# CVlab315/Domain-Adaptative-Hand-Pose-Estimation

Hardware: AMD Instinct MI355X
Metric: images/sec (unique source+target images per A+B+C training iteration, 2*B*N/t_iter) (higher is better)
Workload: dtype bf16; 1 GPU; RHD->H3D domain-adaptation iteration (steps A+B+C), resnet50 + 3-deconv neck + main head + 3 adversarial multiscale-fusion heads, 256x256, batch 64 source + 64 target per GPU, random init, synthetic batches; arch=resnet50, image_size=256, per_gpu_batch=64, global_batch=64, parallelism=dp1, hip_graphs=True, gradient_exchange=none (one rank)

## Files before the change

domain-adaptative-hand-pose-estimation_amd/csrc/conv_plan.h:

```cpp
#pragma once
#include <stdlib.h>
#include "common.h"

#define MAX_TAPS 52
struct Tap { int8_t dy, dx; int16_t widx; };

struct Phase { int OHp, OWp, out_oy, out_ox, M, ntaps, tap0, ntm; };
struct GatherArgs {
  const void* A; const void* B; void* D;
  const float* bias; const void* residual; const float* scale;
  int Hi, Wi, Ci;
  int in_sy, in_sx;
  int Ho, Wo;
  int out_sy, out_sx;
  int Nout, ldb, ldd;
  int cshift;
  int accumulate;
  int nphase, ntn, ntiles;
  int hw;
  int lw;
  unsigned a_bytes, b_bytes;
  size_t stat_bytes;
  int stat_slices;
  const void* bnb_x; const void* bnb_y;
// ... 12 lines not shown
  const float* bias2;
  int c2;
  union { unsigned a2_bytes; unsigned mx_sa_bytes; };
  union { unsigned b2_bytes; unsigned mx_sb_bytes; };
  int pg_nadd;
  int mx_act;
  void* mx_y8; void* mx_sy;
};

inline long conv_knob(const char* name, long dflt, bool* set = nullptr) {
  const char* v = getenv(name);
  if (set) *set = v != nullptr;
  return v ? atol(v) : dflt;
}
inline bool conv_knob_set(const char* name) { bool set; (void)conv_knob(name, 0, &set); return set; }
struct ConvKnobs {
  int tile = (int)conv_knob("MI355_TILE", -1);
  int dma = (int)conv_knob("MI355_DMA", 1);
  int cat_tile = (int)conv_knob("MI355_CAT_TILE", 0);
  int t256d = (int)conv_knob("MI355_T256D", 2);
  long t256d_min = conv_knob("MI355_T256D_MIN", 192);
  long t256d_kmin = conv_knob("MI355_T256D_KMIN", 32);
  bool t256 = conv_knob_set("MI355_T256");
  int kw3 = (int)conv_knob("MI355_KW3", 1);
  int kw3_n64 = (int)conv_knob("MI355_KW3_N64", 1);
  int splitk = (int)conv_knob("MI355_SPLITK", 2);
  long splitk_min = conv_knob("MI355_SPLITK_MIN", 128), splitk_max = conv_knob("MI355_SPLITK_MAX", 320);
  long splitk_kmin = conv_knob("MI355_SPLITK_KMIN", 128);
  bool stats256 = conv_knob("MI355_STATS_256", 1) != 0;
  int phases = (int)conv_knob("MI355_PHASES", 1);
  int wg_blocks = (int)conv_knob("MI355_WG_BLOCKS", 768);
  int wgrad_kw = (int)conv_knob("MI355_WGRAD_KW", 1);
  int wgrad_kw2 = (int)conv_knob("MI355_WGRAD_KW2", 1);
  bool wgrad_group256 = conv_knob("MI355_WGRAD_GROUP256", 1) != 0;
  bool wgrad_kw_group = conv_knob("MI355_WGRAD_KW_GROUP", 1) != 0;
  int wg_group_blocks = (int)conv_knob("MI355_WG_GROUP_BLOCKS", 512);
  int wg_group256_blocks = (int)conv_knob("MI355_WG_GROUP256_BLOCKS", 256);
  int wg_kw_group_blocks = (int)conv_knob("MI355_WG_KW_GROUP_BLOCKS", 512);
  int pgemm = (int)conv_knob("MI355_PGEMM", 1), pgemm_set = -1;
  int pg_add_maxk = (int)conv_knob("MI355_PG_ADD", 1) * 64;
  long pg_min_rows = conv_knob("MI355_PG_MIN_ROWS", 32768);
  int pg_ring = (int)conv_knob("MI355_PG_RING", 0), pg_bm = (int)conv_knob("MI355_PG_BM", 64);
  int pg_per_cu = (int)conv_knob("MI355_PG_PER_CU", 2);
  int fp8_tile = (int)conv_knob("MI355_FP8_TILE", -1);
  long fp8_kw3 = conv_knob("MI355_FP8_KW3", 1024), fp8_kw3_set = -1;
};
inline ConvKnobs& conv_knobs() { static ConvKnobs k; return k; }

static inline void describe_fwd(GatherArgs& a, const mi355_conv_desc* d) {
  a.Hi = d->Hi; a.Wi = d->Wi; a.Ci = d->Ci; a.in_sy = a.in_sx = d->stride;
  a.Ho = d->Ho; a.Wo = d->Wo; a.out_sy = a.out_sx = 1;
  a.Nout = d->Co; a.ldd = d->Co; a.ldb = d->kh * d->kw * d->Ci;
  a.nphase = 1; a.ph[0].OHp = d->Ho; a.ph[0].OWp = d->Wo; a.ph[0].M = d->N * d->Ho * d->Wo; a.ph[0].ntaps = d->kh * d->kw;
  for (int i = 0; i < d->kh; ++i)
    for (int j = 0; j < d->kw; ++j) { Tap& t = a.taps[i * d->kw + j]; t.dy = (int8_t)(i - d->pad); t.dx = (int8_t)(j - d->pad); t.widx = (int16_t)(i * d->kw + j); }
}
static inline bool describe_dgrad(GatherArgs& a, const mi355_conv_desc* d) {
  const int s = d->stride;
  auto parity_without_tap = [&](int k) {
    for (int p = 0; p < s; ++p) { int cnt = 0; for (int i = 0; i < k; ++i) if ((p + d->pad - i) % s == 0) ++cnt; if (!cnt) return true; }
    return false;
  };
  const bool need_zero = parity_without_tap(d->kh) || parity_without_tap(d->kw);
  a.Hi = d->Ho; a.Wi = d->Wo; a.Ci = d->Co;
  a.in_sy = a.in_sx = 1; a.Ho = d->Hi; a.Wo = d->Wi; a.out_sy = a.out_sx = s;
  a.Nout = d->Ci; a.ldd = d->Ci; a.ldb = d->kh * d->kw * d->Co;
// ... 226 lines not shown
constexpr bool gather_has_bnb(int bm, bool hm, bool kw3, bool cat, int kg) { return !hm && bm <= 128 && !kw3 && !cat && kg == 1; }
constexpr bool gather_has_stats(int bm, int bn, bool hm, bool dma) { return !hm && (bm <= 128 || (bm == 256 && bn == 128) || (bm == 256 && bn == 256 && dma)); }
static inline int gather_epilogue(GatherArgs& a, const ConvBuild& b, const ConvKnobs& k) {
  if (!gather_has_bnb(b.bm, b.hm, b.kw3, b.cat, b.kg)) a.bnb_partial = nullptr;
  if (!gather_has_stats(b.bm, b.bn, b.hm, b.dma) || (b.bm == 256 && !k.stats256)) a.stat_partial = nullptr;
  if (!a.stat_partial && !a.bnb_partial) a.stat_slices = 0;
  return a.bnb_partial ? 2 : a.stat_partial ? 1 : 0;
}

static inline void plan_gather_launch(GatherArgs& a, ConvBuild& b, const ConvKnobs& k) {
  plan_tile_grid(a, b.bm, b.bn, b.hm);
  b.epi = b.family == CONV_GATHER ? gather_epilogue(a, b, k) : (b.family == CONV_MX && a.mx_act) ? 3 : (a.stat_partial ? 1 : 0);
  if (b.kw3) a.lw = ilog2_exact(a.Wi);
}

struct WgradSplit { int S, rows; };
static inline WgradSplit wgrad_split(long M, int kstep, long want) {
  const long ksteps = (M + kstep - 1) / kstep;
  long S = want > ksteps ? ksteps : want;
  if (S < 1) S = 1;
  long rps = (M + S - 1) / S; rps = ((rps + kstep - 1) / kstep) * kstep;
  WgradSplit r; r.S = (int)((M + rps - 1) / rps); r.rows = (int)rps;
  return r;
}
static inline WgradSplit wgrad_split_alone(long M, int kstep, long tiles, const ConvKnobs& k) {
  const long ksteps = (M + kstep - 1) / kstep;
  long S = (k.wg_blocks + tiles - 1) / tiles;
  const long S16 = ksteps / 16, S256 = (256 + tiles - 1) / tiles, lo = S16 > S256 ? S16 : S256;
  if (S > lo) S = lo;
  if (tiles >= 384) S = 1;
  return wgrad_split(M, kstep, S);
}

struct WgradPlan { int S, rows_per_split, nto, nti, ldw, kw3, mt, kw2; };
static inline WgradPlan plan_wgrad(const mi355_conv_desc* d, const ConvKnobs& k) {
  WgradPlan w; w.ldw = d->kh * d->kw * d->Ci;
  const int bkm = d->dtype == MI355_BF16 ? 64 : 32;
  const long M = (long)d->N * d->Ho * d->Wo;
  w.kw3 = k.wgrad_kw && d->dtype == MI355_BF16 && d->kh == 3 && d->kw == 3 && d->stride == 1 && d->pad == 1 &&
          d->Ho == d->Hi && d->Wo == d->Wi &&
          d->Wi >= 8 && ilog2_exact(d->Wi) >= 0;
  w.mt = d->Co <= 64 ? 1 : 2;
  w.kw2 = k.wgrad_kw2 && d->dtype == MI355_BF16 && d->kh == d->kw && (d->kh == 3 || d->kh == 4) && d->stride == 2 && d->pad == 1 &&
          d->Hi % 2 == 0 && d->Wi % 2 == 0 && d->Ho == d->Hi / 2 && d->Wo == d->Wi / 2 && d->Wo >= 8 && d->Wo <= 64 &&
          ilog2_exact(d->Wo) >= 0;
  long tiles;
  if (w.kw2) { w.nto = cdiv(d->Co, 64 * w.mt); w.nti = cdiv(d->Ci, 64); tiles = (long)w.nto * d->kh * w.nti; }
  else if (w.kw3) { w.nto = cdiv(d->Co, 64 * w.mt); w.nti = cdiv(d->Ci, 64); tiles = (long)w.nto * 3 * w.nti; }
  else { w.nto = cdiv(d->Co, 128); w.nti = cdiv(w.ldw, 128); tiles = (long)w.nto * w.nti; }
  const WgradSplit s = wgrad_split_alone(M, bkm, tiles, k);
  w.S = s.S; w.rows_per_split = s.rows;
  return w;
}
static inline const char* wgrad_kernel_name(const WgradPlan& w) { return w.kw2 ? "wgrad_kw2" : w.kw3 ? "wgrad_kw" : "wgrad"; }

#define WG_MAX 24
#define WGK_MAX 16
static inline bool group_eligible(const mi355_conv_desc* d, const WgradPlan& w) {
  return !w.kw2 && !w.kw3 && (long)w.nto * w.nti < 384;
}
static inline bool group256_eligible(const mi355_conv_desc* d, const WgradPlan& w) {
  return conv_knobs().wgrad_group256 && d->dtype == MI355_BF16 && d->kh == 1 && d->kw == 1 && d->pad == 0 && d->Co % 256 == 0 && d->Ci % 256 == 0;
}
static inline bool kw_group_eligible(const mi355_conv_desc* d, const WgradPlan& w) {
  if (!conv_knobs().wgrad_kw_group || !w.kw3) return false;
  const long M = (long)d->N * d->Ho * d->Wo, ksteps = (M + 63) / 64;
  return (long)w.nto * 3 * w.nti * ksteps < 768L * 24;
}
static inline long group_tiles(int kind, const mi355_conv_desc* d, const WgradPlan& w) {
  return kind == 3 ? (long)(d->Co / 256) * (w.ldw / 256) : kind == 2 ? (long)w.nto * 3 * w.nti : (long)w.nto * w.nti;
}
struct GroupPlan { int S, rps; size_t ws_off; };
static inline long group_plan(const mi355_wgrad_item* items, const int* idx, int n, GroupPlan* gp, size_t* ws_bytes, int kind) {
  const ConvKnobs& kn = conv_knobs();
  const int target = kind == 3 ? kn.wg_group256_blocks : kind == 2 ? kn.wg_kw_group_blocks : kn.wg_group_blocks;
  auto rows = [](const mi355_conv_desc* d) { return (long)d->N * d->Ho * d->Wo; };
  auto kstep = [](const mi355_conv_desc* d) { return d->dtype == MI355_BF16 ? 64 : 32; };
  double W = 0;
  for (int k = 0; k < n; ++k) {
    const mi355_conv_desc* d = &items[idx[k]].d;
    W += (double)group_tiles(kind, d, plan_wgrad(d, kn)) * ((rows(d) + kstep(d) - 1) / kstep(d));
  }
  long per = (long)(W / target) + 1; if (per < 16) per = 16;
  auto plan_at = [&](long per, GroupPlan* out, size_t* ws_end) {
    long blocks = 0; size_t off = 0;
    for (int k = 0; k < n; ++k) {
      const mi355_wgrad_item& it = items[idx[k]]; const mi355_conv_desc* d = &it.d; const WgradPlan w = plan_wgrad(d, kn);
      const WgradSplit s = wgrad_split(rows(d), kstep(d), ((rows(d) + kstep(d) - 1) / kstep(d) + per - 1) / per);
      if (out) { out[k].S = s.S; out[k].rps = s.rows; out[k].ws_off = off; }
      if (s.S > 1 || it.accumulate) off += (size_t)s.S * d->Co * w.ldw * sizeof(float);
      blocks += group_tiles(kind, d, w) * s.S;
    }
    if (ws_end) *ws_end = off;
    return blocks;
  };
  for (int trial = 0; kind == 3 && trial < 64; ++trial) {
    if (plan_at(per, nullptr, nullptr) <= target) break;
    per += per / 16 + 1;
  }
  return plan_at(per, gp, ws_bytes);
}
template <typename F>
static inline int walk_wgrad_groups(const mi355_wgrad_item* items, int n, F&& fn) {
  int gi[WG_MAX], ki[WGK_MAX], bi[WG_MAX]; int gm = 0, km = 0, bm = 0;
  auto flush_g = [&]() -> int { if (!gm) return 0; int e = fn(1, gi, gm); gm = 0; return e; };
  auto flush_k = [&]() -> int { if (!km) return 0; int e = fn(2, ki, km); km = 0; return e; };
  auto flush_b = [&]() -> int { if (!bm) return 0; int e = fn(3, bi, bm); bm = 0; return e; };
  for (int i = 0; i < n; ++i) {
    const mi355_wgrad_item& it = items[i];
    WgradPlan w = plan_wgrad(&it.d, conv_knobs());
    bool shares = false;
    for (int k = 0; k < gm; ++k) shares = shares || items[gi[k]].dw == it.dw;
    for (int k = 0; k < km; ++k) shares = shares || items[ki[k]].dw == it.dw;
    for (int k = 0; k < bm; ++k) shares = shares || items[bi[k]].dw == it.dw;
    if (shares) { if (int e = flush_g()) return e; if (int e = flush_k()) return e; if (int e = flush_b()) return e; }
    if (kw_group_eligible(&it.d, w)) {
      if (km && (km == WGK_MAX || plan_wgrad(&items[ki[0]].d, conv_knobs()).mt != w.mt)) { if (int e = flush_k()) return e; }
      ki[km++] = i;
    } else if (group_eligible(&it.d, w) && group256_eligible(&it.d, w)) {
      if (bm == WG_MAX) { if (int e = flush_b()) return e; }
      bi[bm++] = i;
    } else if (group_eligible(&it.d, w)) {
      if (gm && (gm == WG_MAX || items[gi[0]].d.dtype != it.d.dtype)) { if (int e = flush_g()) return e; }
      gi[gm++] = i;
    } else {
      int one = i;
      if (int e = fn(0, &one, 1)) return e;
    }
  }
  if (int e = flush_g()) return e;
  if (int e = flush_b()) return e;
  return flush_k();
}
```

domain-adaptative-hand-pose-estimation_amd/csrc/igemm.hip:

```cpp
#include "common.h"
#include <stdlib.h>

#include "igemm_common.h"

template <typename T> struct MmaTraits;
template <> struct MmaTraits<bf16_t> { static constexpr int BK = 64; static constexpr int CH = 8; };
template <> struct MmaTraits<float> { static constexpr int BK = 32; static constexpr int CH = 4; };

#define GATHER_STAGES 1
template <typename T, int BM, int BN, int STAGES = 1, bool KW3 = false>
struct GatherSmem {
  static constexpr int kARows = KW3 ? BM + 4 * (BM / 8) + 4 : BM;
  static constexpr int kStage = (kARows + BN) * 128;
  static constexpr int kOutStride = BN * (int)sizeof(T) + 16;
  static constexpr int kOut = BM * kOutStride;
  static constexpr int kBytes = (STAGES * kStage > kOut ? STAGES * kStage : kOut) + BM * 4;
};

template <typename T, int BM, int BN, bool SMALL_C, int WGM = 2, int WGN = 2, bool HM_OUT = false, bool DMA = false, int EPI = 0,
          bool KW3 = false, bool CAT = false, int KG = 1>
__global__ __launch_bounds__(64 * WGM * WGN * KG, (KW3 && BM == 256) ? 2 : 1) void gather_gemm_kernel(const GatherArgs p) {
  constexpr int CH = MmaTraits<T>::CH;
  constexpr int GTHR = 64 * WGM * WGN;
  constexpr int NTHR = GTHR * KG, RPP = GTHR / 8;
// ... 829 lines not shown
    const unsigned st = smem_lds + (unsigned)((it & 1) * STAGE);
    __builtin_amdgcn_s_setprio(1);
    wg256_step<0>(st, trA, trB, acc); wg256_step<4096>(st, trA, trB, acc); wg256_step<8192>(st, trA, trB, acc); wg256_step<12288>(st, trA, trB, acc);
    __builtin_amdgcn_s_setprio(0);
  }
  float* out = p.out + (size_t)split * p.slab_stride;
#pragma unroll
  for (int i = 0; i < 4; ++i)
#pragma unroll
    for (int j = 0; j < 2; ++j)
#pragma unroll
      for (int r = 0; r < 16; ++r) {
        const int o = o0 + wo * 128 + i * 32 + (r & 3) + 8 * (r >> 2) + 4 * hi;
        const int c = c0 + (wc >> 1) * 128 + wn0 + j * 32 + r31;
        if (o < p.Co && c < p.ldw) out[(size_t)o * p.ldw + c] = acc[i][j][r];
      }
}
__global__ __launch_bounds__(512, 1) void wgrad_group256_kernel(const WgradGroupArgs g) {
  extern __shared__ __attribute__((aligned(16))) char smem256[];
  int i = 0;
  while (i + 1 < g.n && (int)blockIdx.x >= g.bstart[i + 1]) ++i;
  wgrad_gemm256_body(g.p[i], (int)blockIdx.x - g.bstart[i], g.bstart[i + 1] - g.bstart[i], smem256);
}

struct SlabItem { const float* slabs; float* out; long n4, stride; int S, accumulate; };
struct SlabGroupArgs { SlabItem it[WG_MAX]; int bstart[WG_MAX + 1]; int n; };
__global__ __launch_bounds__(256) void slab_reduce_group_kernel(const SlabGroupArgs g) {
  int i = 0;
  while (i + 1 < g.n && (int)blockIdx.x >= g.bstart[i + 1]) ++i;
  const SlabItem& q = g.it[i];
  const long c = (long)((int)blockIdx.x - g.bstart[i]) * 256 + threadIdx.x;
  if (c >= q.n4) return;
  float4 v = make_float4(0.f, 0.f, 0.f, 0.f);
  for (int s = 0; s < q.S; ++s) {
    const float4 a = reinterpret_cast<const float4*>(q.slabs + (size_t)s * q.stride)[c];
    v.x += a.x; v.y += a.y; v.z += a.z; v.w += a.w;
  }
  if (q.accumulate) { const float4 o = reinterpret_cast<const float4*>(q.out)[c]; v.x += o.x; v.y += o.y; v.z += o.z; v.w += o.w; }
  reinterpret_cast<float4*>(q.out)[c] = v;
}

struct WgradKwArgs {
  const void* X; const void* DY; float* out;
  int H, W, Ci, Co;
  int lw, lwf, halo;
  int M, rows_per_split, ldw;
  long slab_stride;
  int nto, nci;
  unsigned x_bytes, dy_bytes;
  FastDiv dH;
};
__device__ __forceinline__ int swzx(int r, int ch) { return r * 128 + ((ch ^ (((r >> 1) & 1) << 2)) << 4); }

template <int MT> struct WgradKwSmem { static constexpr int kBytes = 64 * 256 + (64 + 4 * 8 + 4) * 128 + 2 * 64 * 4; };
template <int MT>
__device__ __forceinline__ void wgrad_kw_body(const WgradKwArgs& p, const int bid, const int nblk, char* smem) {
  constexpr int BO = 64 * MT, BKM = 64;
  constexpr int CPRY = BO / 8, RPY = 256 / CPRY, NPY = BKM / RPY;
  constexpr int XROWS = 64 + 4 * 8 + 4;
  char* ys = smem;
  char* xs = smem + BKM * 256;
  int* rowinfo = reinterpret_cast<int*>(smem + BKM * 256 + XROWS * 128);

  const int t = threadIdx.x, lane = t & 63, wave = t >> 6;
  const int ntile = p.nto * 3 * p.nci;
  const int lid = xcd_remap(bid, nblk);
  const int split = lid / ntile;
// ... 103 lines not shown
        b[k] = __builtin_shufflevector(b0, b1, 0, 1, 2, 3, 4, 5, 6, 7);
      }
#pragma unroll
      for (int k = 0; k < 3; ++k)
#pragma unroll
        for (int i = 0; i < MT; ++i) acc[k][i] = __builtin_amdgcn_mfma_f32_32x32x16_bf16(a[i], b[k], acc[k][i], 0, 0, 0);
    }
    __builtin_amdgcn_s_setprio(0);
  }
  float* out = p.out + (size_t)split * p.slab_stride;
#pragma unroll
  for (int k = 0; k < 3; ++k)
#pragma unroll
    for (int i = 0; i < MT; ++i)
#pragma unroll
      for (int r = 0; r < 16; ++r) {
        const int o = o0 + wm0 + i * 32 + (r & 3) + 8 * (r >> 2) + 4 * hi;
        const int c = ci0 + wn0 + r31;
        if (o < p.Co && c < p.Ci) out[(size_t)o * p.ldw + (kh * 3 + k) * p.Ci + c] = acc[k][i][r];
      }
}
template <int MT>
__global__ __launch_bounds__(256, 3) void wgrad_kw_kernel(const WgradKwArgs p) {
  __shared__ __attribute__((aligned(16))) char smem[WgradKwSmem<MT>::kBytes];
  wgrad_kw_body<MT>(p, (int)blockIdx.x, (int)gridDim.x, smem);
}
struct WgradKwGroupArgs { WgradKwArgs p[WGK_MAX]; int bstart[WGK_MAX + 1]; int n; };
template <int MT>
__global__ __launch_bounds__(256, 3) void wgrad_kw_group_kernel(const WgradKwGroupArgs g) {
  __shared__ __attribute__((aligned(16))) char smem[WgradKwSmem<MT>::kBytes];
  int i = 0;
  while (i + 1 < g.n && (int)blockIdx.x >= g.bstart[i + 1]) ++i;
  wgrad_kw_body<MT>(g.p[i], (int)blockIdx.x - g.bstart[i], g.bstart[i + 1] - g.bstart[i], smem);
}

struct WgradKw2Args {
  const void* X; const void* DY; float* out;
  int H, W, Ho, Ci, Co;
  int lw, lwo;
  int M, rows_per_split, ldw;
  long slab_stride;
  int nto, nci;
  unsigned x_bytes, dy_bytes;
  FastDiv dHo;
};

template <int MT, int KW>
__global__ __launch_bounds__(256, KW == 4 ? 2 : 3) void wgrad_kw2_kernel(const WgradKw2Args p) {
  constexpr int BO = 64 * MT, BKM = 64;
  constexpr int CPRY = BO / 8, RPY = 256 / CPRY, NPY = BKM / RPY;
  constexpr int XROWS = 64 + 4 * 8 + 4;
  __shared__ __attribute__((aligned(16))) char smem[BKM * 256 + 2 * XROWS * 128 + 2 * BKM * 8];
  char* ys = smem;
  char* xe = smem + BKM * 256;
  char* xo = xe + XROWS * 128;
  int2* rowinfo = reinterpret_cast<int2*>(smem + BKM * 256 + 2 * XROWS * 128);

  const int t = threadIdx.x, lane = t & 63, wave = t >> 6;
  const int ntile = p.nto * KW * p.nci;
  const int lid = xcd_remap(blockIdx.x, gridDim.x);
  const int split = lid / ntile;
  int tile = lid - split * ntile;
  const int ot = tile / (KW * p.nci); tile -= ot * KW * p.nci;
  const int kh = tile / p.nci, cit = tile - kh * p.nci;
  const int o0 = ot * BO, ci0 = cit * 64, tdy = kh - 1;
  const int wm0 = (wave >> 1) * (32 * MT), wn0 = (wave & 1) * 32;
// ... 558 lines not shown
}
static int check_wgrad_channels(const mi355_conv_desc* d) {
  const int CH = d->dtype == MI355_BF16 ? 8 : 4;
  if (d->Ci % CH || d->Co % CH) MI_FAIL(MI355_EINVAL, "wgrad: channels must be multiples of %d", CH);
  if (ilog2_exact(d->Ci / CH) < 0) MI_FAIL(MI355_EINVAL, "wgrad: Ci/%d must be a power of two", CH);
  return MI355_OK;
}

extern "C" size_t mi355_conv_wgrad_workspace(const mi355_conv_desc* d) {
  WgradPlan w = plan_wgrad(d, conv_knobs());
  return (size_t)w.S * d->Co * w.ldw * sizeof(float);
}

extern "C" int mi355_conv_wgrad(const mi355_conv_desc* d, const void* x, const void* dy, float* dw, int accumulate,
                                void* ws, size_t ws_bytes, void* stream) {
  if (int e = check_desc(d, true)) return e;
  hipStream_t st = as_stream(stream);
  if (int e = check_wgrad_channels(d)) return e;
  const WgradPlan w = plan_wgrad(d, conv_knobs());
  const size_t need = (size_t)w.S * d->Co * w.ldw * sizeof(float);
  const bool direct = (w.S == 1 && !accumulate);
  if (!direct && (ws == nullptr || ws_bytes < need)) MI_FAIL(MI355_EWORKSPACE, "wgrad workspace %zu < %zu", ws_bytes, need);
  float* out = direct ? dw : reinterpret_cast<float*>(ws);
  const long M = (long)d->N * d->Ho * d->Wo, slab = (long)d->Co * w.ldw, esz = d->dtype == MI355_BF16 ? 2 : 4;
  const unsigned x_bytes = (unsigned)((long)d->N * d->Hi * d->Wi * d->Ci * esz), dy_bytes = (unsigned)(M * d->Co * esz);
  {
    if (prof_on()) prof_set_tag("%s k%ds%d %d>%d @%dx%d n%d S%d", wgrad_kernel_name(w), d->kh, d->stride, d->Ci, d->Co, d->Hi, d->Wi, d->N, w.S);
    ProfScope ps(st, 2.0 * M * (double)d->Co * w.ldw, (double)x_bytes + (double)dy_bytes + 4.0 * d->Co * w.ldw);
    if (w.kw2) {
      WgradKw2Args k; fill_wgrad_args(k, d, w, x, dy, out, w.rows_per_split);
      dim3 grid(w.nto * d->kh * w.nti * w.S);
      if (d->kh == 3) { if (w.mt == 1) hipLaunchKernelGGL((wgrad_kw2_kernel<1, 3>), grid, dim3(256), 0, st, k); else hipLaunchKernelGGL((wgrad_kw2_kernel<2, 3>), grid, dim3(256), 0, st, k); }
      else { if (w.mt == 1) hipLaunchKernelGGL((wgrad_kw2_kernel<1, 4>), grid, dim3(256), 0, st, k); else hipLaunchKernelGGL((wgrad_kw2_kernel<2, 4>), grid, dim3(256), 0, st, k); }
    } else if (w.kw3) {
      WgradKwArgs k; fill_wgrad_args(k, d, w, x, dy, out, w.rows_per_split);
      dim3 grid(w.nto * 3 * w.nti * w.S);
      if (w.mt == 1) hipLaunchKernelGGL(wgrad_kw_kernel<1>, grid, dim3(256), 0, st, k);
      else hipLaunchKernelGGL(wgrad_kw_kernel<2>, grid, dim3(256), 0, st, k);
    } else {
      WgradArgs a; fill_wgrad_args(a, d, w, x, dy, out, w.rows_per_split);
      dim3 grid(w.nto * w.nti * w.S);
      if (d->dtype == MI355_BF16) hipLaunchKernelGGL(wgrad_gemm_kernel<bf16_t>, grid, dim3(256), 0, st, a);
      else hipLaunchKernelGGL(wgrad_gemm_kernel<float>, grid, dim3(256), 0, st, a);
    }
    MI_CHECK_LAUNCH(wgrad_kernel_name(w));
  }
  if (!direct) {
    launch_slab_reduce(reinterpret_cast<const float*>(ws), dw, slab, w.S, slab, accumulate, st);
    MI_CHECK_LAUNCH("slab_reduce");
  }
  return MI355_OK;
}


static void slab_group_add(SlabGroupArgs& sg, int& nblocks, const float* slabs, float* out, long slab_stride, int S, int accumulate) {
  SlabItem& q = sg.it[sg.n];
  q.slabs = slabs; q.out = out; q.n4 = slab_stride / 4; q.stride = slab_stride; q.S = S; q.accumulate = accumulate;
  sg.bstart[sg.n] = nblocks; nblocks += cdiv(q.n4, 256); ++sg.n;
}
static int launch_slab_reduce_group(SlabGroupArgs& sg, int nblocks, hipStream_t st) {
  sg.bstart[sg.n] = nblocks;
  if (!sg.n) return MI355_OK;
  double sb = 0; for (int k = 0; k < sg.n; ++k) sb += 16.0 * sg.it[k].n4 * (sg.it[k].S + 1);
  char lab[64];
  if (prof_on()) snprintf(lab, sizeof(lab), "slab_reduce_group x%d", sg.n);
  ProfScope ps(st, 0.0, sb, 2, prof_on() ? lab : nullptr);
  hipLaunchKernelGGL(slab_reduce_group_kernel, dim3(nblocks), dim3(256), 0, st, sg); MI_CHECK_LAUNCH("slab_reduce_group");
  return MI355_OK;
}
extern "C" size_t mi355_conv_wgrad_grouped_workspace(const mi355_wgrad_item* items, int n) {
  if (!items || n < 1) return 0;
  size_t need = 0;
  (void)walk_wgrad_groups(items, n, [&](int kind, const int* idx, int m) -> int {
    size_t b = 0;
    if (kind == 0) b = mi355_conv_wgrad_workspace(&items[idx[0]].d);
    else { static_assert(WGK_MAX <= WG_MAX, "one plan array for every kind"); GroupPlan gp[WG_MAX]; group_plan(items, idx, m, gp, &b, kind); }
    if (b > need) need = b;
    return 0;
  });
  return need;
}
static void launch_group_kernel(const WgradGroupArgs& g, int nb, int kind, const mi355_conv_desc* d0, hipStream_t st) {
  if (kind == 3) {
    static bool attr_set = false;
    if (!attr_set) { (void)hipFuncSetAttribute((const void*)wgrad_group256_kernel, hipFuncAttributeMaxDynamicSharedMemorySize, WG256_SMEM); attr_set = true; }
    hipLaunchKernelGGL(wgrad_group256_kernel, dim3(nb), dim3(512), WG256_SMEM, st, g);
  }
  else if (d0->dtype == MI355_BF16) hipLaunchKernelGGL(wgrad_group_kernel<bf16_t>, dim3(nb), dim3(256), 0, st, g);
  else hipLaunchKernelGGL(wgrad_group_kernel<float>, dim3(nb), dim3(256), 0, st, g);
}
static void launch_group_kernel(const WgradKwGroupArgs& g, int nb, int, const mi355_conv_desc* d0, hipStream_t st) {
  if (plan_wgrad(d0, conv_knobs()).mt == 1) hipLaunchKernelGGL(wgrad_kw_group_kernel<1>, dim3(nb), dim3(256), 0, st, g);
  else hipLaunchKernelGGL(wgrad_kw_group_kernel<2>, dim3(nb), dim3(256), 0, st, g);
}
template <typename Group>
static int launch_wgrad_group(const mi355_wgrad_item* items, const int* idx, int n, void* ws, size_t ws_bytes, hipStream_t st, int kind) {
  const char* name = kind == 3 ? "wgrad_group256" : kind == 2 ? "wgrad_kw_group" : "wgrad_group";
  GroupPlan gp[WG_MAX]; size_t need = 0;
  group_plan(items, idx, n, gp, &need, kind);
  if (need && (!ws || ws_bytes < need)) MI_FAIL(MI355_EWORKSPACE, "%s workspace %zu < %zu", name, ws_bytes, need);
  Group g; memset(&g, 0, sizeof(g));
  SlabGroupArgs sg; memset(&sg, 0, sizeof(sg));
  int nb = 0, nsb = 0;
  double flops = 0, bytes = 0;
  for (int k = 0; k < n; ++k) {
    const mi355_wgrad_item& it = items[idx[k]]; const mi355_conv_desc* d = &it.d;
    if (kind != 2) { if (int e = check_wgrad_channels(d)) return e; }
    WgradPlan w = plan_wgrad(d, conv_knobs());
    if (kind == 3) { w.nto = d->Co / 256; w.nti = w.ldw / 256; }
    const bool direct = gp[k].S == 1 && !it.accumulate;
    auto& a = g.p[k];
    fill_wgrad_args(a, d, w, it.x, it.dy, direct ? it.dw : reinterpret_cast<float*>(reinterpret_cast<char*>(ws) + gp[k].ws_off), gp[k].rps);
    g.bstart[k] = nb; nb += (int)group_tiles(kind, d, w) * gp[k].S;
    flops += 2.0 * a.M * (double)d->Co * w.ldw; bytes += (double)a.x_bytes + a.dy_bytes + 4.0 * d->Co * w.ldw;
    if (!direct) slab_group_add(sg, nsb, a.out, it.dw, a.slab_stride, gp[k].S, it.accumulate);
  }
  g.bstart[n] = nb; g.n = n;
  {
    const mi355_conv_desc* d0 = &items[idx[0]].d;
    if (prof_on()) prof_set_tag("%s x%d blocks%d first k%ds%d %d>%d @%dx%d", name, n, nb, d0->kh, d0->stride, d0->Ci, d0->Co, d0->Hi, d0->Wi);
    ProfScope ps(st, flops, bytes);
    launch_group_kernel(g, nb, kind, d0, st);
    MI_CHECK_LAUNCH(name);
  }
  return launch_slab_reduce_group(sg, nsb, st);
}
extern "C" int mi355_conv_wgrad_grouped(const mi355_wgrad_item* items, int n, void* ws, size_t ws_bytes, void* stream) {
  if (!items || n < 1) MI_FAIL(MI355_EINVAL, "wgrad_grouped: no items");
  hipStream_t st = as_stream(stream);
  for (int i = 0; i < n; ++i) {
    if (int e = check_desc(&items[i].d)) return e;
    if (!items[i].x || !items[i].dy || !items[i].dw) MI_FAIL(MI355_EINVAL, "wgrad_grouped: item %d has a null operand", i);
  }
  return walk_wgrad_groups(items, n, [&](int kind, const int* idx, int m) -> int {
    if (kind == 0) { const mi355_wgrad_item& it = items[idx[0]]; return mi355_conv_wgrad(&it.d, it.x, it.dy, it.dw, it.accumulate, ws, ws_bytes, stream); }
    if (kind == 2) return launch_wgrad_group<WgradKwGroupArgs>(items, idx, m, ws, ws_bytes, st, kind);
    return launch_wgrad_group<WgradGroupArgs>(items, idx, m, ws, ws_bytes, st, kind);
  });
}

template <typename T>
__global__ void pack_weights_kernel(const float* __restrict__ w, T* __restrict__ wf, T* __restrict__ wt, int O, int Tt, int I, int Ipad) {
  __shared__ float tile[32][33];
  const int tap = blockIdx.z, o0 = blockIdx.y * 32, i0 = blockIdx.x * 32;
  const int tx = threadIdx.x & 31, ty = threadIdx.x >> 5;
  for (int r = ty; r < 32; r += 8) {
    int o = o0 + r, i = i0 + tx;
    float v = (o < O && i < I) ? w[((size_t)o * Tt + tap) * I + i] : 0.f;
    tile[r][tx] = v;
    if (wf && o < O && i < Ipad) Elem<T>::st(wf + ((size_t)o * Tt + tap) * Ipad + i, v);
  }
  __syncthreads();
  if (wt)
    for (int r = ty; r < 32; r += 8) {
      int i = i0 + r, o = o0 + tx;
      if (o < O && i < Ipad) Elem<T>::st(wt + ((size_t)i * Tt + tap) * O + o, tile[tx][r]);
    }
}

template <typename T>
__global__ void pack_weights_batched_kernel(const mi355_pack_item* __restrict__ items, int nitems) {
  __shared__ float tile[32][33];
  int lo = 0, hi = nitems - 1;
  const int b = blockIdx.x;
  while (lo < hi) { const int mid = (lo + hi + 1) >> 1; if (items[mid].blk0 <= b) lo = mid; else hi = mid - 1; }
  const mi355_pack_item it = items[lo];
  const int O = it.O, Tt = it.T, I = it.I, Ipad = it.Ipad;
  const int nbi = (Ipad + 31) / 32, nbo = (O + 31) / 32;
  int q = b - it.blk0;
// ... 39 lines not shown
```

profiles/insitu_table.py:

```python
import csv
import json
import re
import sys
import collections

trace, logf, iters = sys.argv[1], sys.argv[2], int(sys.argv[3])
MFMA, HBM = 1.75e15, 6.3e12

PAT = [('fwd8', 'gather_fp8_kernel'), ('dgrad8', 'gather_fp8_kernel'), ('fwd', ('gather_gemm_kernel', 'pgemm_kernel')),
       ('dgrad', ('gather_gemm_kernel', 'pgemm_kernel')), ('hm1x1', 'gather_gemm_kernel'), ('wgrad_kw_group', 'wgrad_kw_group_kernel'),
       ('wgrad_kw2', 'wgrad_kw2_kernel'), ('wgrad_kw', 'wgrad_kw_kernel'), ('wgrad_group256', 'wgrad_group256_kernel'), ('wgrad_group', 'wgrad_group_kernel'),
       ('wgrad8', 'wgrad_kw'), ('wgrad', 'wgrad_gemm_kernel'),
       ('bn_stats', 'bn_stats_kernel'), ('bn_finalize', 'bn_finalize'), ('bn_apply', 'bn_apply_kernel'), ('bn_relu_maxpool', 'bn_relu_maxpool_kernel'),
       ('bn_bwd_res', 'bn_bwd_resident_kernel'), ('bn_bwd_reduce', 'bn_bwd_reduce_kernel'), ('bn_bwd_finalize', 'bn_bwd_finalize_kernel'),
       ('bn_bwd_apply', 'bn_bwd_apply_kernel'), ('slab_reduce_group', 'slab_reduce_group_kernel'), ('slab_reduce', 'slab_reduce_kernel')]
FAMILY_KERNELS = {0: ('gather_gemm_kernel', 'gather_fp8_kernel', 'pgemm_kernel', 'wgrad_gemm_kernel', 'wgrad_kw_kernel', 'wgrad_kw2_kernel',
                      'wgrad_group_kernel', 'wgrad_group256_kernel', 'wgrad_kw_group_kernel', 'wgrad_kw8_kernel', 'wgrad_kw28_kernel'),
                  1: ('bn_stats_kernel', 'bn_finalize_kernel', 'bn_finalize_wide_kernel', 'bn_apply_kernel', 'bn_relu_maxpool_kernel',
                      'bn_bwd_resident_kernel', 'bn_bwd_reduce_kernel', 'bn_bwd_finalize_kernel', 'bn_bwd_apply_kernel'),
                  2: ('slab_reduce_kernel', 'slab_reduce_group_kernel')}


def base(name):
    m = re.match(r'_Z\d+([A-Za-z0-9_]+?)I', name)
    if m:
        return m.group(1)
    return re.sub(r'<.*|\(.*', '', re.sub(r'^void ', '', name)).strip()


log = json.load(open(logf))['launches']
rows = []
for r in csv.DictReader(open(trace)):
    rows.append((int(r['Start_Timestamp']), base(r['Kernel_Name']), r['Kernel_Name'], (int(r['End_Timestamp']) - int(r['Start_Timestamp'])) / 1e3,
                 int(r['Grid_Size_X']) // max(int(r['Workgroup_Size_X']), 1)))
rows.sort()
out = []
for fam in (0, 1, 2):
    ents = [e for e in log if e['family'] == fam]
    if not ents:
        continue
    ks = [r for r in rows if r[1] in FAMILY_KERNELS[fam]]
    if fam == 1:
        ks = [r for r in ks if not (r[1] == 'bn_bwd_reduce_kernel' and 'Lb0ELi0E' in r[2])]
    n = len(ents)
    if len(ks) < n * iters:
        print('# family %d: trace holds %d launches, fewer than %d x %d -- skipped' % (fam, len(ks), iters, n)); continue
    ks = ks[-n * iters:]
    bad = 0
    for j, e in enumerate(ents):
        want = next((k for p, k in PAT if e['label'].startswith(p)), '?')
# ... 33 lines not shown
```

profiles/pmc_fold.py:

```python
import collections
import csv
import gzip
import json
import os
import re
import sys

FAMILIES = [
    ('conv_mfma', ('gather_gemm_kernel', 'wgrad_gemm_kernel', 'wgrad_kw_kernel', 'wgrad_kw2_kernel', 'wgrad_kw_group_kernel', 'gather_fp8_kernel', 'pgemm_kernel',
                   'wgrad_group_kernel', 'wgrad_group256_kernel', 'wgrad_kw8_kernel', 'wgrad_kw28_kernel')),
    ('slab_reduce', ('slab_reduce_kernel', 'slab_reduce_group_kernel')),
    ('bn_fwd', ('bn_stats_kernel', 'bn_apply_kernel', 'bn_finalize_kernel', 'bn_finalize_wide_kernel', 'bn_relu_maxpool_kernel')),
    ('bn_bwd', ('bn_bwd_resident_kernel', 'bn_bwd_reduce_kernel', 'bn_bwd_apply_kernel', 'bn_bwd_finalize_kernel')),
    ('kl_loss', ('kl_heatmap_kernel', 'kl_heatmap_reg_kernel')),
    ('argmax', ('argmax2d_kernel', 'argmax2d_reg_kernel')),
    ('softargmax', ('softargmax_kernel', 'softargmax_reg_kernel')),
    ('pseudo_label', ('pseudo_label_kernel', 'pseudo_label_reg_kernel')),
    ('pointwise21', ('pw_k2c', 'pw_c2k', 'pw_wgrad', 'hm_rowsum')),
    ('fp8_quantize', ('quantize_fp8_kernel', 'pack_weights_fp8_kernel', 'fp8_update_scale_kernel')),
    ('optimizer', ('sgd_kernel', 'pack_weights')),
    ('pool_layout', ('maxpool', 'nchw_to_nhwc', 'nhwc_to_nchw')),
]


def family(name):
    for fam, keys in FAMILIES:
        if any(k in name for k in keys):
            return fam
    return 'other'


def _open(path):
    return gzip.open(path, 'rt') if path.endswith('.gz') else open(path)


def fold_counter(path, counter):
    acc = collections.defaultdict(lambda: [0, 0.0])
    with _open(path) as f:
        for r in csv.DictReader(f):
            if r['Counter_Name'] != counter:
                continue
            a = acc[r['Kernel_Name']]
            a[0] += 1
# ... 60 lines not shown
```

Before: 4295 images/s.

## Add 3x3 weight-gradient kernel computing all nine taps per 64x64 tile

Result: no change. 4335 images/s, median of 6 (+0.9%).

```diff
diff --git a/domain-adaptative-hand-pose-estimation_amd/csrc/conv_plan.h b/domain-adaptative-hand-pose-estimation_amd/csrc/conv_plan.h
--- a/domain-adaptative-hand-pose-estimation_amd/csrc/conv_plan.h
+++ b/domain-adaptative-hand-pose-estimation_amd/csrc/conv_plan.h
@@ -68,6 +68,7 @@
   int wg_blocks = (int)conv_knob("MI355_WG_BLOCKS", 768);
   int wgrad_kw = (int)conv_knob("MI355_WGRAD_KW", 1);
   int wgrad_kw2 = (int)conv_knob("MI355_WGRAD_KW2", 1);
+  int wgrad_k9 = (int)conv_knob("MI355_WGRAD_K9", 1);
   bool wgrad_group256 = conv_knob("MI355_WGRAD_GROUP256", 1) != 0;
   bool wgrad_kw_group = conv_knob("MI355_WGRAD_KW_GROUP", 1) != 0;
   int wg_group_blocks = (int)conv_knob("MI355_WG_GROUP_BLOCKS", 512);
@@ -360,7 +361,8 @@
   return wgrad_split(M, kstep, S);
 }
 
-struct WgradPlan { int S, rows_per_split, nto, nti, ldw, kw3, mt, kw2; };
+struct WgradPlan { int S, rows_per_split, nto, nti, ldw, kw3, mt, kw2, k9; };
+static inline long wgrad_kw_tiles(const mi355_conv_desc* d) { return (long)cdiv(d->Co, d->Co <= 64 ? 64 : 128) * 3 * cdiv(d->Ci, 64); }
 static inline WgradPlan plan_wgrad(const mi355_conv_desc* d, const ConvKnobs& k) {
   WgradPlan w; w.ldw = d->kh * d->kw * d->Ci;
   const int bkm = d->dtype == MI355_BF16 ? 64 : 32;
@@ -369,18 +371,22 @@
           d->Ho == d->Hi && d->Wo == d->Wi &&
           d->Wi >= 8 && ilog2_exact(d->Wi) >= 0;
   w.mt = d->Co <= 64 ? 1 : 2;
+  w.k9 = w.kw3 && k.wgrad_k9 && d->Ci == d->Co && d->Ci % 64 == 0 && d->Wi <= 64 &&
+         (k.wgrad_k9 >= 2 || (M >= 4096 && d->Ci >= 128 && d->Wi >= 16));
+  if (w.k9) w.mt = 1;
   w.kw2 = k.wgrad_kw2 && d->dtype == MI355_BF16 && d->kh == d->kw && (d->kh == 3 || d->kh == 4) && d->stride == 2 && d->pad == 1 &&
           d->Hi % 2 == 0 && d->Wi % 2 == 0 && d->Ho == d->Hi / 2 && d->Wo == d->Wi / 2 && d->Wo >= 8 && d->Wo <= 64 &&
           ilog2_exact(d->Wo) >= 0;
   long tiles;
   if (w.kw2) { w.nto = cdiv(d->Co, 64 * w.mt); w.nti = cdiv(d->Ci, 64); tiles = (long)w.nto * d->kh * w.nti; }
+  else if (w.k9) { w.nto = d->Co / 64; w.nti = d->Ci / 64; tiles = wgrad_kw_tiles(d); }
   else if (w.kw3) { w.nto = cdiv(d->Co, 64 * w.mt); w.nti = cdiv(d->Ci, 64); tiles = (long)w.nto * 3 * w.nti; }
   else { w.nto = cdiv(d->Co, 128); w.nti = cdiv(w.ldw, 128); tiles = (long)w.nto * w.nti; }
   const WgradSplit s = wgrad_split_alone(M, bkm, tiles, k);
   w.S = s.S; w.rows_per_split = s.rows;
   return w;
 }
-static inline const char* wgrad_kernel_name(const WgradPlan& w) { return w.kw2 ? "wgrad_kw2" : w.kw3 ? "wgrad_kw" : "wgrad"; }
+static inline const char* wgrad_kernel_name(const WgradPlan& w) { return w.kw2 ? "wgrad_kw2" : w.k9 ? "wgrad_k9" : w.kw3 ? "wgrad_kw" : "wgrad"; }
 
 #define WG_MAX 24
 #define WGK_MAX 16
@@ -393,7 +399,7 @@
 static inline bool kw_group_eligible(const mi355_conv_desc* d, const WgradPlan& w) {
   if (!conv_knobs().wgrad_kw_group || !w.kw3) return false;
   const long M = (long)d->N * d->Ho * d->Wo, ksteps = (M + 63) / 64;
-  return (long)w.nto * 3 * w.nti * ksteps < 768L * 24;
+  return wgrad_kw_tiles(d) * ksteps < 768L * 24;
 }
 static inline long group_tiles(int kind, const mi355_conv_desc* d, const WgradPlan& w) {
   return kind == 3 ? (long)(d->Co / 256) * (w.ldw / 256) : kind == 2 ? (long)w.nto * 3 * w.nti : (long)w.nto * w.nti;
@@ -401,13 +407,13 @@
 struct GroupPlan { int S, rps; size_t ws_off; };
 static inline long group_plan(const mi355_wgrad_item* items, const int* idx, int n, GroupPlan* gp, size_t* ws_bytes, int kind) {
   const ConvKnobs& kn = conv_knobs();
-  const int target = kind == 3 ? kn.wg_group256_blocks : kind == 2 ? kn.wg_kw_group_blocks : kn.wg_group_blocks;
+  const int target = kind == 3 ? kn.wg_group256_blocks : (kind == 2 || kind == 4) ? kn.wg_kw_group_blocks : kn.wg_group_blocks;
   auto rows = [](const mi355_conv_desc* d) { return (long)d->N * d->Ho * d->Wo; };
   auto kstep = [](const mi355_conv_desc* d) { return d->dtype == MI355_BF16 ? 64 : 32; };
   double W = 0;
   for (int k = 0; k < n; ++k) {
     const mi355_conv_desc* d = &items[idx[k]].d;
-    W += (double)group_tiles(kind, d, plan_wgrad(d, kn)) * ((rows(d) + kstep(d) - 1) / kstep(d));
+    W += (double)(kind == 4 ? wgrad_kw_tiles(d) : group_tiles(kind, d, plan_wgrad(d, kn))) * ((rows(d) + kstep(d) - 1) / kstep(d));
   }
   long per = (long)(W / target) + 1; if (per < 16) per = 16;
   auto plan_at = [&](long per, GroupPlan* out, size_t* ws_end) {
@@ -430,10 +436,11 @@
 }
 template <typename F>
 static inline int walk_wgrad_groups(const mi355_wgrad_item* items, int n, F&& fn) {
-  int gi[WG_MAX], ki[WGK_MAX], bi[WG_MAX]; int gm = 0, km = 0, bm = 0;
+  int gi[WG_MAX], ki[WGK_MAX], bi[WG_MAX], ni[WGK_MAX]; int gm = 0, km = 0, bm = 0, nm = 0;
   auto flush_g = [&]() -> int { if (!gm) return 0; int e = fn(1, gi, gm); gm = 0; return e; };
   auto flush_k = [&]() -> int { if (!km) return 0; int e = fn(2, ki, km); km = 0; return e; };
   auto flush_b = [&]() -> int { if (!bm) return 0; int e = fn(3, bi, bm); bm = 0; return e; };
+  auto flush_n = [&]() -> int { if (!nm) return 0; int e = fn(4, ni, nm); nm = 0; return e; };
   for (int i = 0; i < n; ++i) {
     const mi355_wgrad_item& it = items[i];
     WgradPlan w = plan_wgrad(&it.d, conv_knobs());
@@ -441,8 +448,12 @@
     for (int k = 0; k < gm; ++k) shares = shares || items[gi[k]].dw == it.dw;
     for (int k = 0; k < km; ++k) shares = shares || items[ki[k]].dw == it.dw;
     for (int k = 0; k < bm; ++k) shares = shares || items[bi[k]].dw == it.dw;
-    if (shares) { if (int e = flush_g()) return e; if (int e = flush_k()) return e; if (int e = flush_b()) return e; }
-    if (kw_group_eligible(&it.d, w)) {
+    for (int k = 0; k < nm; ++k) shares = shares || items[ni[k]].dw == it.dw;
+    if (shares) { if (int e = flush_g()) return e; if (int e = flush_k()) return e; if (int e = flush_b()) return e; if (int e = flush_n()) return e; }
+    if (kw_group_eligible(&it.d, w) && w.k9) {
+      if (nm && (nm == WGK_MAX || (items[ni[0]].d.Co <= 64) != (it.d.Co <= 64))) { if (int e = flush_n()) return e; }
+      ni[nm++] = i;
+    } else if (kw_group_eligible(&it.d, w)) {
       if (km && (km == WGK_MAX || plan_wgrad(&items[ki[0]].d, conv_knobs()).mt != w.mt)) { if (int e = flush_k()) return e; }
       ki[km++] = i;
     } else if (group_eligible(&it.d, w) && group256_eligible(&it.d, w)) {
@@ -458,5 +469,6 @@
   }
   if (int e = flush_g()) return e;
   if (int e = flush_b()) return e;
-  return flush_k();
-}
+  if (int e = flush_k()) return e;
+  return flush_n();
+}
diff --git a/domain-adaptative-hand-pose-estimation_amd/csrc/igemm.hip b/domain-adaptative-hand-pose-estimation_amd/csrc/igemm.hip
--- a/domain-adaptative-hand-pose-estimation_amd/csrc/igemm.hip
+++ b/domain-adaptative-hand-pose-estimation_amd/csrc/igemm.hip
@@ -885,7 +885,15 @@
   const long c = (long)((int)blockIdx.x - g.bstart[i]) * 256 + threadIdx.x;
   if (c >= q.n4) return;
   float4 v = make_float4(0.f, 0.f, 0.f, 0.f);
-  for (int s = 0; s < q.S; ++s) {
+  int s = 0;
+  for (; s + 7 < q.S; s += 8) {
+    float4 a[8];
+#pragma unroll
+    for (int u = 0; u < 8; ++u) a[u] = reinterpret_cast<const float4*>(q.slabs + (size_t)(s + u) * q.stride)[c];
+#pragma unroll
+    for (int u = 0; u < 8; ++u) { v.x += a[u].x; v.y += a[u].y; v.z += a[u].z; v.w += a[u].w; }
+  }
+  for (; s < q.S; ++s) {
     const float4 a = reinterpret_cast<const float4*>(q.slabs + (size_t)s * q.stride)[c];
     v.x += a.x; v.y += a.y; v.z += a.z; v.w += a.w;
   }
@@ -1055,6 +1063,160 @@
   int i = 0;
   while (i + 1 < g.n && (int)blockIdx.x >= g.bstart[i + 1]) ++i;
   wgrad_kw_body<MT>(g.p[i], (int)blockIdx.x - g.bstart[i], g.bstart[i + 1] - g.bstart[i], smem);
+}
+
+template <int LW> struct WgradK9Cfg {
+  static constexpr int W = 1 << LW, R = 64 / W, NSLOT = R + 2 <= 4 ? 4 : R + 2 <= 8 ? 8 : 16;
+  static constexpr int SEG = (W + 4) * 128, ZOFF = NSLOT * SEG, XBYTES = (NSLOT + 1) * SEG;
+};
+constexpr int kWgradK9Smem = 64 * 256 + WgradK9Cfg<6>::XBYTES;
+static_assert(WgradK9Cfg<3>::XBYTES <= WgradK9Cfg<6>::XBYTES && WgradK9Cfg<4>::XBYTES <= WgradK9Cfg<6>::XBYTES &&
+              WgradK9Cfg<5>::XBYTES <= WgradK9Cfg<6>::XBYTES, "the W = 64 image is the largest");
+template <int LW>
+__device__ __forceinline__ void wgrad_k9_body(const WgradKwArgs& p, const int bid, const int nblk, char* smem) {
+  typedef WgradK9Cfg<LW> C;
+  constexpr int W = C::W, BKM = 64;
+  constexpr int AHEAD = 1;
+  char* ys = smem;
+  char* xs = smem + BKM * 256;
+
+  const int t = threadIdx.x, lane = t & 63, wave = t >> 6;
+  const int ntile = p.nto * p.nci;
+  const int lid = xcd_remap(bid, nblk);
+  const int split = lid / ntile;
+  const int tile = lid - split * ntile;
+  const int ot = tile / p.nci, cit = tile - ot * p.nci;
+  const int o0 = ot * 64, ci0 = cit * 64;
+  const int wm0 = (wave >> 1) * 32, wn0 = (wave & 1) * 32;
+
+  const __amdgpu_buffer_rsrc_t rsX = make_rsrc(p.X, p.x_bytes), rsY = make_rsrc(p.DY, p.dy_bytes);
+  const int lc = t & 7, lr = t >> 3;
+  const int mbeg = split * p.rows_per_split;
+  const int mend = min(p.M, mbeg + p.rows_per_split);
+  const int g0 = mbeg >> LW;
+  auto xaddr = [&](int m, int ch) { return swzx((((m >> LW) - g0 + 1) & (C::NSLOT - 1)) * (W + 4) + 2 + (m & (W - 1)), ch); };
+
+  for (int i = t; i < C::XBYTES / 16; i += 256) reinterpret_cast<uint4*>(xs)[i] = make_uint4(0, 0, 0, 0);
+  __syncthreads();
+  for (int j = t; j < 2 * W * 8; j += 256) {
+    const int m = mbeg - W + (j >> 3), ch = j & 7;
+    const uint4 v = buf_load16(rsX, (m >= 0 && m < p.M) ? (m * p.Ci + ci0 + ch * 8) * 2 : OOB_OFF);
+    *reinterpret_cast<uint4*>(xs + xaddr(m, ch)) = v;
+  }
+
+  uint4 ry[2], rx[2];
+  auto load_tile = [&](int mt0) {
+#pragma unroll
+    for (int i = 0; i < 2; ++i) {
+      const int m = mt0 + lr + 32 * i;
+      ry[i] = buf_load16(rsY, m < mend ? (m * p.Co + o0 + lc * 8) * 2 : OOB_OFF);
+    }
+#pragma unroll
+    for (int i = 0; i < 2; ++i) {
+      const int m = mt0 + W + lr + 32 * i;
+      rx[i] = buf_load16(rsX, m < p.M ? (m * p.Ci + ci0 + lc * 8) * 2 : OOB_OFF);
+    }
+  };
+  auto store_tile = [&](int mt0) {
+#pragma unroll
+    for (int i = 0; i < 2; ++i) *reinterpret_cast<uint4*>(ys + swz256(lr + 32 * i, lc)) = ry[i];
+#pragma unroll
+    for (int i = 0; i < 2; ++i) *reinterpret_cast<uint4*>(xs + xaddr(mt0 + W + lr + 32 * i, lc)) = rx[i];
+  };
+
+  f32x16_t acc[9];
+#pragma unroll
+  for (int a = 0; a < 9; ++a)
+#pragma unroll
+    for (int r = 0; r < 16; ++r) acc[a][r] = 0.f;
+
+  const int r31 = lane & 31, hi = lane >> 5;
+  const int tg = lane >> 4, tq = (lane & 15) >> 2, tp = lane & 3;
+  int trA[2], trB[3][2];
+#pragma unroll
+  for (int u = 0; u < 2; ++u) {
+    const int row = 8 * (tg >> 1) + tq + 4 * u;
+    trA[u] = swz256(row, wm0 / 8 + 2 * (tg & 1) + (tp >> 1)) + 8 * (tp & 1);
+#pragma unroll
+    for (int a = 0; a < 3; ++a) trB[a][u] = swzx(1 + (row & (W - 1)) + a, wn0 / 8 + 2 * (tg & 1) + (tp >> 1)) + 8 * (tp & 1);
+  }
+  if (mbeg < mend) load_tile(mbeg);
+  for (int mt0 = mbeg; mt0 < mend; mt0 += BKM) {
+    __syncthreads();
+    store_tile(mt0);
+    __syncthreads();
+    if (mt0 + BKM < mend) load_tile(mt0 + BKM);
+    const int rrel = (mt0 >> LW) - g0;
+    __builtin_amdgcn_s_setprio(1);
+    typedef __attribute__((address_space(3))) bf16x4_t* lds4;
+    int sbase[4][3];
+    bf16x8_t a[4];
+#pragma unroll
+    for (int s = 0; s < 4; ++s) {
+      const int seg = ((16 * s) >> LW) + (LW == 3 ? hi : 0);
+      const unsigned g = (unsigned)((mt0 >> LW) + seg);
+      const int oy = (int)(g - fd_div(g, p.dH) * (unsigned)p.H);
+      const bool past = mt0 + 16 * s + (LW == 3 ? 8 * hi : 0) >= p.M;
+      const int xoff = ((16 * s) & (W - 1)) * 128;
+#pragma unroll
+      for (int kh = 0; kh < 3; ++kh) {
+        int base = ((rrel + seg + kh) & (C::NSLOT - 1)) * C::SEG;
+        if (kh == 0) base = oy == 0 ? C::ZOFF : base;
+        if (kh == 2) base = oy == p.H - 1 ? C::ZOFF : base;
+        sbase[s][kh] = (past ? C::ZOFF : base) + xoff;
+      }
+      bf16x4_t a0 = __builtin_amdgcn_ds_read_tr16_b64_v4i16((lds4)(ys + trA[0] + s * 4096));
+      bf16x4_t a1 = __builtin_amdgcn_ds_read_tr16_b64_v4i16((lds4)(ys + trA[1] + s * 4096));
+      a[s] = __builtin_shufflevector(a0, a1, 0, 1, 2, 3, 4, 5, 6, 7);
+    }
+    bf16x8_t b[AHEAD + 1][3];
+    auto read_frag = [&](int g, int kw) {
+      bf16x4_t b0 = __builtin_amdgcn_ds_read_tr16_b64_v4i16((lds4)(xs + sbase[g / 3][g % 3] + trB[kw][0]));
+      bf16x4_t b1 = __builtin_amdgcn_ds_read_tr16_b64_v4i16((lds4)(xs + sbase[g / 3][g % 3] + trB[kw][1]));
+      return (bf16x8_t)__builtin_shufflevector(b0, b1, 0, 1, 2, 3, 4, 5, 6, 7);
+    };
+#pragma unroll
+    for (int g = 0; g < AHEAD; ++g)
+#pragma unroll
+      for (int kw = 0; kw < 3; ++kw) b[g][kw] = read_frag(g, kw);
+#pragma unroll
+    for (int g = 0; g < 12; ++g)
+#pragma unroll
+      for (int kw = 0; kw < 3; ++kw) {
+        if (g + AHEAD < 12) b[(g + AHEAD) % (AHEAD + 1)][kw] = read_frag(g + AHEAD, kw);
+        __builtin_amdgcn_sched_barrier(0);
+        acc[(g % 3) * 3 + kw] = __builtin_amdgcn_mfma_f32_32x32x16_bf16(a[g / 3], b[g % (AHEAD + 1)][kw], acc[(g % 3) * 3 + kw], 0, 0, 0);
+        __builtin_amdgcn_sched_barrier(0);
+      }
+    __builtin_amdgcn_s_setprio(0);
+  }
+  float* out = p.out + (size_t)split * p.slab_stride;
+#pragma unroll
+  for (int k = 0; k < 9; ++k)
+#pragma unroll
+    for (int r = 0; r < 16; ++r) {
+      const int o = o0 + wm0 + (r & 3) + 8 * (r >> 2) + 4 * hi;
+      const int c = ci0 + wn0 + r31;
+      out[(size_t)o * p.ldw + k * p.Ci + c] = acc[k][r];
+    }
+}
+__device__ __forceinline__ void wgrad_k9_any(const WgradKwArgs& p, const int bid, const int nblk, char* smem) {
+  switch (p.lw) {
+    case 3: wgrad_k9_body<3>(p, bid, nblk, smem); break;
+    case 4: wgrad_k9_body<4>(p, bid, nblk, smem); break;
+    case 5: wgrad_k9_body<5>(p, bid, nblk, smem); break;
+    default: wgrad_k9_body<6>(p, bid, nblk, smem); break;
+  }
+}
+__global__ __launch_bounds__(256, 2) void wgrad_k9_kernel(const WgradKwArgs p) {
+  __shared__ __attribute__((aligned(16))) char smem[kWgradK9Smem];
+  wgrad_k9_any(p, (int)blockIdx.x, (int)gridDim.x, smem);
+}
+__global__ __launch_bounds__(256, 2) void wgrad_k9_group_kernel(const WgradKwGroupArgs g) {
+  __shared__ __attribute__((aligned(16))) char smem[kWgradK9Smem];
+  int i = 0;
+  while (i + 1 < g.n && (int)blockIdx.x >= g.bstart[i + 1]) ++i;
+  wgrad_k9_any(g.p[i], (int)blockIdx.x - g.bstart[i], g.bstart[i + 1] - g.bstart[i], smem);
 }
 
 struct WgradKw2Args {
@@ -1679,6 +1841,9 @@
       dim3 grid(w.nto * d->kh * w.nti * w.S);
       if (d->kh == 3) { if (w.mt == 1) hipLaunchKernelGGL((wgrad_kw2_kernel<1, 3>), grid, dim3(256), 0, st, k); else hipLaunchKernelGGL((wgrad_kw2_kernel<2, 3>), grid, dim3(256), 0, st, k); }
       else { if (w.mt == 1) hipLaunchKernelGGL((wgrad_kw2_kernel<1, 4>), grid, dim3(256), 0, st, k); else hipLaunchKernelGGL((wgrad_kw2_kernel<2, 4>), grid, dim3(256), 0, st, k); }
+    } else if (w.k9) {
+      WgradKwArgs k; fill_wgrad_args(k, d, w, x, dy, out, w.rows_per_split);
+      hipLaunchKernelGGL(wgrad_k9_kernel, dim3(w.nto * w.nti * w.S), dim3(256), 0, st, k);
     } else if (w.kw3) {
       WgradKwArgs k; fill_wgrad_args(k, d, w, x, dy, out, w.rows_per_split);
       dim3 grid(w.nto * 3 * w.nti * w.S);
@@ -1736,13 +1901,14 @@
   else if (d0->dtype == MI355_BF16) hipLaunchKernelGGL(wgrad_group_kernel<bf16_t>, dim3(nb), dim3(256), 0, st, g);
   else hipLaunchKernelGGL(wgrad_group_kernel<float>, dim3(nb), dim3(256), 0, st, g);
 }
-static void launch_group_kernel(const WgradKwGroupArgs& g, int nb, int, const mi355_conv_desc* d0, hipStream_t st) {
-  if (plan_wgrad(d0, conv_knobs()).mt == 1) hipLaunchKernelGGL(wgrad_kw_group_kernel<1>, dim3(nb), dim3(256), 0, st, g);
+static void launch_group_kernel(const WgradKwGroupArgs& g, int nb, int kind, const mi355_conv_desc* d0, hipStream_t st) {
+  if (kind == 4) hipLaunchKernelGGL(wgrad_k9_group_kernel, dim3(nb), dim3(256), 0, st, g);
+  else if (plan_wgrad(d0, conv_knobs()).mt == 1) hipLaunchKernelGGL(wgrad_kw_group_kernel<1>, dim3(nb), dim3(256), 0, st, g);
   else hipLaunchKernelGGL(wgrad_kw_group_kernel<2>, dim3(nb), dim3(256), 0, st, g);
 }
 template <typename Group>
 static int launch_wgrad_group(const mi355_wgrad_item* items, const int* idx, int n, void* ws, size_t ws_bytes, hipStream_t st, int kind) {
-  const char* name = kind == 3 ? "wgrad_group256" : kind == 2 ? "wgrad_kw_group" : "wgrad_group";
+  const char* name = kind == 4 ? "wgrad_k9_group" : kind == 3 ? "wgrad_group256" : kind == 2 ? "wgrad_kw_group" : "wgrad_group";
   GroupPlan gp[WG_MAX]; size_t need = 0;
   group_plan(items, idx, n, gp, &need, kind);
   if (need && (!ws || ws_bytes < need)) MI_FAIL(MI355_EWORKSPACE, "%s workspace %zu < %zu", name, ws_bytes, need);
@@ -1752,7 +1918,7 @@
   double flops = 0, bytes = 0;
   for (int k = 0; k < n; ++k) {
     const mi355_wgrad_item& it = items[idx[k]]; const mi355_conv_desc* d = &it.d;
-    if (kind != 2) { if (int e = check_wgrad_channels(d)) return e; }
+    if (kind != 2 && kind != 4) { if (int e = check_wgrad_channels(d)) return e; }
     WgradPlan w = plan_wgrad(d, conv_knobs());
     if (kind == 3) { w.nto = d->Co / 256; w.nti = w.ldw / 256; }
     const bool direct = gp[k].S == 1 && !it.accumulate;
@@ -1781,7 +1947,7 @@
   }
   return walk_wgrad_groups(items, n, [&](int kind, const int* idx, int m) -> int {
     if (kind == 0) { const mi355_wgrad_item& it = items[idx[0]]; return mi355_conv_wgrad(&it.d, it.x, it.dy, it.dw, it.accumulate, ws, ws_bytes, stream); }
-    if (kind == 2) return launch_wgrad_group<WgradKwGroupArgs>(items, idx, m, ws, ws_bytes, st, kind);
+    if (kind == 2 || kind == 4) return launch_wgrad_group<WgradKwGroupArgs>(items, idx, m, ws, ws_bytes, st, kind);
     return launch_wgrad_group<WgradGroupArgs>(items, idx, m, ws, ws_bytes, st, kind);
   });
 }
diff --git a/profiles/insitu_table.py b/profiles/insitu_table.py
--- a/profiles/insitu_table.py
+++ b/profiles/insitu_table.py
@@ -9,13 +9,14 @@
 
 PAT = [('fwd8', 'gather_fp8_kernel'), ('dgrad8', 'gather_fp8_kernel'), ('fwd', ('gather_gemm_kernel', 'pgemm_kernel')),
        ('dgrad', ('gather_gemm_kernel', 'pgemm_kernel')), ('hm1x1', 'gather_gemm_kernel'), ('wgrad_kw_group', 'wgrad_kw_group_kernel'),
+       ('wgrad_k9_group', 'wgrad_k9_group_kernel'), ('wgrad_k9', 'wgrad_k9_kernel'),
        ('wgrad_kw2', 'wgrad_kw2_kernel'), ('wgrad_kw', 'wgrad_kw_kernel'), ('wgrad_group256', 'wgrad_group256_kernel'), ('wgrad_group', 'wgrad_group_kernel'),
        ('wgrad8', 'wgrad_kw'), ('wgrad', 'wgrad_gemm_kernel'),
        ('bn_stats', 'bn_stats_kernel'), ('bn_finalize', 'bn_finalize'), ('bn_apply', 'bn_apply_kernel'), ('bn_relu_maxpool', 'bn_relu_maxpool_kernel'),
        ('bn_bwd_res', 'bn_bwd_resident_kernel'), ('bn_bwd_reduce', 'bn_bwd_reduce_kernel'), ('bn_bwd_finalize', 'bn_bwd_finalize_kernel'),
        ('bn_bwd_apply', 'bn_bwd_apply_kernel'), ('slab_reduce_group', 'slab_reduce_group_kernel'), ('slab_reduce', 'slab_reduce_kernel')]
 FAMILY_KERNELS = {0: ('gather_gemm_kernel', 'gather_fp8_kernel', 'pgemm_kernel', 'wgrad_gemm_kernel', 'wgrad_kw_kernel', 'wgrad_kw2_kernel',
-                      'wgrad_group_kernel', 'wgrad_group256_kernel', 'wgrad_kw_group_kernel', 'wgrad_kw8_kernel', 'wgrad_kw28_kernel'),
+                      'wgrad_group_kernel', 'wgrad_group256_kernel', 'wgrad_kw_group_kernel', 'wgrad_k9_kernel', 'wgrad_k9_group_kernel', 'wgrad_kw8_kernel', 'wgrad_kw28_kernel'),
                   1: ('bn_stats_kernel', 'bn_finalize_kernel', 'bn_finalize_wide_kernel', 'bn_apply_kernel', 'bn_relu_maxpool_kernel',
                       'bn_bwd_resident_kernel', 'bn_bwd_reduce_kernel', 'bn_bwd_finalize_kernel', 'bn_bwd_apply_kernel'),
                   2: ('slab_reduce_kernel', 'slab_reduce_group_kernel')}
diff --git a/profiles/pmc_fold.py b/profiles/pmc_fold.py
--- a/profiles/pmc_fold.py
+++ b/profiles/pmc_fold.py
@@ -8,7 +8,7 @@
 
 FAMILIES = [
     ('conv_mfma', ('gather_gemm_kernel', 'wgrad_gemm_kernel', 'wgrad_kw_kernel', 'wgrad_kw2_kernel', 'wgrad_kw_group_kernel', 'gather_fp8_kernel', 'pgemm_kernel',
-                   'wgrad_group_kernel', 'wgrad_group256_kernel', 'wgrad_kw8_kernel', 'wgrad_kw28_kernel')),
+                   'wgrad_group_kernel', 'wgrad_group256_kernel', 'wgrad_kw8_kernel', 'wgrad_kw28_kernel', 'wgrad_k9_kernel', 'wgrad_k9_group_kernel')),
     ('slab_reduce', ('slab_reduce_kernel', 'slab_reduce_group_kernel')),
     ('bn_fwd', ('bn_stats_kernel', 'bn_apply_kernel', 'bn_finalize_kernel', 'bn_finalize_wide_kernel', 'bn_relu_maxpool_kernel')),
     ('bn_bwd', ('bn_bwd_resident_kernel', 'bn_bwd_reduce_kernel', 'bn_bwd_apply_kernel', 'bn_bwd_finalize_kernel')),
```
